# yg838457845/ORB_SLAM2-Chinese-annotation

Measured on AMD Instinct MI355X. Metric: frames/sec (extract+match) at 1241×376, 1000 feat/frame; 1/2/4/8 GPU, higher is better.
Workload: dtype u8; 1 GPU; C4: 1241x376 KITTI-shaped synthetic stream, 1000 feat/frame, SearchByProjection vs 5000-point local map per frame; distinct_frames_per_gpu=8192, frames_per_launch=1024, parallelism=single rank; no collective (one process, one GPU)

## Files before the change

orb_slam2-chinese-annotation_amd/csrc/matcher_kernels.hip:

```cpp
#include <algorithm>
#include <cmath>

#include "matcher_common.h"

__global__ __launch_bounds__(256) void k_hamming_batch(const uint8_t* __restrict__ a,
                                                       const uint8_t* __restrict__ b, int n,
                                                       int32_t* __restrict__ out) {
  const int i = blockIdx.x * blockDim.x + threadIdx.x;
  if (i >= n) return;
  out[i] = hamming256(load_desc(a + (size_t)i * 32), load_desc(b + (size_t)i * 32));
}

#define GB_LDS_KEYS 8192
__global__ __launch_bounds__(64) void k_grid_build(const orb_keypoint_t* __restrict__ keys,
                                                   const int32_t* __restrict__ nkeys, int kpStride,
                                                   float minX, float minY, float invW, float invH,
                                                   int32_t* __restrict__ cellStart,
                                                   int32_t* __restrict__ cellIdx,
                                                   const uint8_t* __restrict__ locked,
                                                   const float* __restrict__ uright,
                                                   uint4* __restrict__ staged) {
  __shared__ __attribute__((aligned(16))) int cnt[GRID_CELLS + 4];
  const int p = blockIdx.x, lane = threadIdx.x;
  const int n = max(nkeys[p], 0);
// ... 361 lines not shown
#pragma unroll
      for (int k = 1; k < 4; ++k)
        if (ix0 + k > nMaxCellX) len[k] = 0;
      const int c1 = len[0], c2 = c1 + len[1], c3 = c2 + len[2], total = c3 + len[3];
      const int o1 = lo[1] - c1, o2 = lo[2] - c2, o3 = lo[3] - c3;
      for (int t = 0; t < total; ++t) {
        const int j = t + (t < c1 ? lo[0] : t < c2 ? o1 : t < c3 ? o2 : o3);
        const uint4 E = gKp[j];
        const int oct = (int)((E.z >> 24) & 0x7Fu);
        if (oct < minL || oct > maxL) continue;
        const float dx = __uint_as_float(E.x) - x, dy = __uint_as_float(E.y) - y;
        if (!(fabsf(dx) < rs && fabsf(dy) < rs) || (E.z >> 31) != 0) continue;
        const float ur = __uint_as_float(E.w);
        if (ur > 0 && fabsf(mp.proj_xr - ur) > rs) continue;
        fn((E.z & 0xFFFFFFu) | ((uint32_t)oct << 24));
      }
    }
  };
  if (staged) {
    int nq = 0;
    uint32_t qe[PROJ_QB];
#pragma unroll
    for (int k = 0; k < PROJ_QB; ++k) qe[k] = 0;
    auto flush = [&](int cnt) {
      ulonglong4 dd[PROJ_QB];
#pragma unroll
      for (int k = 0; k < PROJ_QB; ++k)
        dd[k] = load_desc(D + (size_t)((k < cnt ? qe[k] : qe[0]) & 0xFFFFFFu) * 32);
#pragma unroll
      for (int k = 0; k < PROJ_QB; ++k) {
        if (k >= cnt) break;
        const int dist = hamming256(q, dd[k]);
        if (dist >= 256) continue;
        ++count;
        top.insert(pack_cand((int)(qe[k] & 0xFFFFFFu), dist, (int)(qe[k] >> 24)), dist);
      }
    };
    walk([&](uint32_t qv) {
#pragma unroll
      for (int k = 0; k < PROJ_QB; ++k) qe[k] = nq == k ? qv : qe[k];
      if (++nq == PROJ_QB) {
        flush(PROJ_QB);
        nq = 0;
      }
    });
    if (nq) flush(nq);
  } else {
    for_features_in_area(K, cs, ci, P, mp.proj_x, mp.proj_y, rs, lvl - 1, lvl,
                         [&](int idx, const orb_keypoint_t& kp) {
                           visit(idx, kp.octave, LK && LK[idx], UR ? UR[idx] : -1.0f);
                         });
  }
  top.store(topk + mg * TOPK);
  int slot = -1;
  if (count > TOPK && count <= OVF_CAP && P.ovf) {
    slot = ovf_alloc(P.ovfCtr + p, P.gen);
    if (slot >= OVF_SLOTS) slot = -1;
  }
  if (slot >= 0) {
    uint32_t* lst = P.ovf + ((size_t)p * OVF_SLOTS + slot) * OVF_CAP;
    int n = 0;
    auto put = [&](int idx, int oct) {
      const int dist = hamming256(q, load_desc(D + (size_t)idx * 32));
      if (dist < 256 && n < OVF_CAP) lst[n++] = pack_cand(idx, dist, oct);
    };
    if (staged)
      walk([&](uint32_t qv) { put((int)(qv & 0xFFFFFFu), (int)(qv >> 24)); });
    else
      for_features_in_area(K, cs, ci, P, mp.proj_x, mp.proj_y, rs, lvl - 1, lvl,
                           [&](int idx, const orb_keypoint_t& kp) {
                             if ((LK && LK[idx]) || (UR && UR[idx] > 0 && fabsf(mp.proj_xr - UR[idx]) > rs))
                               return;
                             put(idx, kp.octave);
                           });
  }
  ncand[mg] = count | (mp.has_obs ? NC_OBS : 0) | ((slot + 1) << NC_SLOT_SHIFT);
  }
}

__device__ __forceinline__ bool lock_test(const uint32_t* bm, int idx) {
  return (bm[idx >> 5] >> (idx & 31)) & 1u;
}


template <int NW>
__global__ __launch_bounds__(64 * NW) void k_proj_resolve(
    const orb_keypoint_t* __restrict__ keys, const uint8_t* __restrict__ desc,
    const float* __restrict__ uright, const uint8_t* __restrict__ locked,
    const int32_t* __restrict__ nkeys, int kpStride, const orb_mp_track_t* __restrict__ mps,
    const uint8_t* __restrict__ mpDesc, const int32_t* __restrict__ nmps, int mpStride,
    const int32_t* __restrict__ cellStart, const int32_t* __restrict__ cellIdx, ProjParams P,
    const uint32_t* __restrict__ topk, const int32_t* __restrict__ ncand,
    int32_t* __restrict__ kpMatch, int32_t* __restrict__ nmatches) {
  constexpr int W = 64 * NW, CHUNK = 256 * NW;
  extern __shared__ __attribute__((aligned(16))) uint32_t dyn[];
  __shared__ uint4 cTop[CHUNK];
  __shared__ int cN[CHUNK];
  __shared__ uint8_t cObs[CHUNK];
  __shared__ int sFirst[NW], sCount[NW];
  __shared__ int sSlow;
  const int p = blockIdx.x, t = threadIdx.x, lane = t & 63, wv = t >> 6;
  const int n = nkeys[p], M = nmps[p];
  const int words = (kpStride + 31) >> 5;
  uint32_t* bm = dyn;
  int* claimBy = (int*)(dyn + ((words + 3) & ~3));
  for (int i = t; i < words; i += W) bm[i] = 0u;
  for (int i = t; i < kpStride; i += W) claimBy[i] = W;
  int32_t* km = kpMatch + (size_t)p * kpStride;
  for (int i = t; i < n; i += W) km[i] = -1;
  __syncthreads();
  const float nnratio = P.nnratio;
  const size_t pbase = (size_t)p * mpStride;
  int matches = 0;
  int start = 0;
  int cb = -CHUNK;
  while (start < M) {
    if (start + W > cb + CHUNK && cb + CHUNK < M) {
      cb = start;
      __syncthreads();
      for (int j = t; j < CHUNK; j += W) {
        const int m = cb + j;
        if (m < M) {
          cTop[j] = *reinterpret_cast<const uint4*>(topk + (pbase + m) * TOPK);
          const int v = ncand[pbase + m];
          cN[j] = v;
          cObs[j] = nc_obs(v);
        }
      }
      __syncthreads();
    }
    const int m = start + t;
    const bool active = m < M;
    int nc = -1, ncRaw = -1;
    uint32_t e[TOPK];
    bool hasObs = false;
    if (active) {
      const int j = m - cb;
      ncRaw = cN[j];
      nc = nc_count(ncRaw);
      const uint4 t4 = cTop[j];
      e[0] = t4.x; e[1] = t4.y; e[2] = t4.z; e[3] = t4.w;
      hasObs = cObs[j] != 0;
    }
    int bestDist = 256, bestLevel = -1, bestDist2 = 256, bestLevel2 = -1, bestIdx = -1;
    int consumed = 0, found = 0;
    if (nc > 0) {
      const int avail = nc < TOPK ? nc : TOPK;
      for (int j = 0; j < avail && found < 2; ++j) {
        ++consumed;
        const int idx = cand_idx(e[j]);
        if (lock_test(bm, idx)) continue;
        if (found == 0) {
          bestDist = cand_dist(e[j]);
          bestLevel = cand_oct(e[j]);
          bestIdx = idx;
        } else {
          bestDist2 = cand_dist(e[j]);
          bestLevel2 = cand_oct(e[j]);
        }
        ++found;
      }
    }
    const bool slow = nc > TOPK && found < 2;
    const int slowSlot = nc_slot(ncRaw);
    bool accept = false;
    if (nc > 0 && !slow && bestDist <= 100)
      accept = !(bestLevel == bestLevel2 && (float)bestDist > nnratio * (float)bestDist2);
    const bool locks = accept && hasObs;
    if (locks) atomicMin(&claimBy[bestIdx], t);
    __syncthreads();
    bool conflict = false;
    for (int q = 0; q < consumed; ++q) conflict |= claimBy[cand_idx(e[q])] < t;
    const unsigned long long bad = __ballot(active && (conflict || (slow && t > 0)));
    if (lane == 0) sFirst[wv] = bad ? wv * 64 + (int)__builtin_ctzll(bad) : W;
    if (t == 0) sSlow = active && slow;
    __syncthreads();
    if (locks) claimBy[bestIdx] = W;
    int commit = W;
#pragma unroll
    for (int i = 0; i < NW; ++i) commit = min(commit, sFirst[i]);
    if (sSlow) {
      if (t == 0 && slowSlot >= 0) {
        const uint32_t* lst = ovf_list(P, p, slowSlot);
        int bd = 256, bl = -1, bd2 = 256, bl2 = -1, bi = -1;
        for (int j = 0; j < nc; ++j) {
          const uint32_t ce = lst[j];
          const int idx = cand_idx(ce);
          if (lock_test(bm, idx)) continue;
          const int dist = cand_dist(ce);
          if (dist < bd) {
            bd2 = bd; bd = dist; bl2 = bl; bl = cand_oct(ce); bi = idx;
          } else if (dist < bd2) {
            bl2 = cand_oct(ce); bd2 = dist;
          }
        }
        if (bd <= 100 && !(bl == bl2 && (float)bd > nnratio * (float)bd2)) {
          atomicMax(&km[bi], m);
          if (cObs[m - cb]) bm[bi >> 5] |= 1u << (bi & 31);
          ++matches;
        }
      } else if (t == 0) {
        const size_t mg = pbase + m;
        const orb_mp_track_t mp = mps[mg];
        const int lvl = mp.level;
        float r = (double)mp.view_cos > 0.998 ? 2.5f : 4.0f;
        if (P.th != 1.0f) r *= P.th;
        const float rs = r * P.scale[lvl];
        const orb_keypoint_t* K = keys + (size_t)p * kpStride;
        const uint8_t* D = desc + (size_t)p * kpStride * 32;
        const uint8_t* LK = locked ? locked + (size_t)p * kpStride : nullptr;
        const float* UR = uright ? uright + (size_t)p * kpStride : nullptr;
        const ulonglong4 qd = load_desc(mpDesc + mg * 32);
        int bd = 256, bl = -1, bd2 = 256, bl2 = -1, bi = -1;
        for_features_in_area(K, cellStart + (size_t)p * (GRID_CELLS + 1),
                             cellIdx + (size_t)p * kpStride, P, mp.proj_x, mp.proj_y, rs,
                             lvl - 1, lvl, [&](int idx, const orb_keypoint_t& kp) {
                               if ((LK && LK[idx]) || lock_test(bm, idx)) return;
                               if (UR && UR[idx] > 0) {
                                 const float er = fabsf(mp.proj_xr - UR[idx]);
                                 if (er > r * P.scale[lvl]) return;
                               }
                               const int dist = hamming256(qd, load_desc(D + (size_t)idx * 32));
                               if (dist < bd) {
                                 bd2 = bd; bd = dist; bl2 = bl; bl = kp.octave; bi = idx;
                               } else if (dist < bd2) {
                                 bl2 = kp.octave; bd2 = dist;
                               }
                             });
        if (bd <= 100 && !(bl == bl2 && (float)bd > nnratio * (float)bd2)) {
          atomicMax(&km[bi], m);
          if (mp.has_obs) bm[bi >> 5] |= 1u << (bi & 31);
          ++matches;
        }
      }
      commit = 1;
    } else {
      if (t < commit && accept) {
        atomicMax(&km[bestIdx], m);
        if (locks) atomicOr(&bm[bestIdx >> 5], 1u << (bestIdx & 31));
      }
      matches += __popcll(__ballot(t < commit && accept));
    }
    __syncthreads();
    start += commit;
  }
  if (lane == 0) sCount[wv] = matches;
  __syncthreads();
  if (t == 0) {
    int tot = 0;
#pragma unroll
    for (int i = 0; i < NW; ++i) tot += sCount[i];
    nmatches[p] = tot;
  }
}


__device__ __forceinline__ void lds_barrier() {
  __builtin_amdgcn_fence(__ATOMIC_RELEASE, "workgroup", "local");
  __builtin_amdgcn_s_barrier();
  __builtin_amdgcn_fence(__ATOMIC_ACQUIRE, "workgroup", "local");
}

__device__ __noinline__ int fp_slow(int m, const int* cur, const orb_mp_track_t* mpp,
                                    const uint8_t* mpd, const orb_keypoint_t* K, const uint8_t* D,
                                    const uint8_t* LK, const float* UR, const int32_t* cs,
                                    const int32_t* ci, const ProjParams P, const uint32_t* lst,
                                    int nl) {
  if (lst) {
    uint32_t e[OVF_CAP];
#pragma unroll
    for (int j = 0; j < OVF_CAP; j += 4) {
      const uint4 v = *reinterpret_cast<const uint4*>(lst + j);
      e[j] = v.x; e[j + 1] = v.y; e[j + 2] = v.z; e[j + 3] = v.w;
    }
    int cv[OVF_CAP];
#pragma unroll
    for (int j = 0; j < OVF_CAP; ++j) cv[j] = cur[cand_idx(j < nl ? e[j] : e[0])];
    int bestDist = 256, bestLevel = -1, bestDist2 = 256, bestLevel2 = -1, bestIdx = -1;
#pragma unroll
    for (int j = 0; j < OVF_CAP; ++j) {
      if (j >= nl || cv[j] < m) continue;
      const int dist = cand_dist(e[j]);
      if (dist < bestDist) {
        bestDist2 = bestDist; bestDist = dist;
        bestLevel2 = bestLevel; bestLevel = cand_oct(e[j]); bestIdx = cand_idx(e[j]);
      } else if (dist < bestDist2) {
        bestLevel2 = cand_oct(e[j]); bestDist2 = dist;
      }
    }
    const bool accept = bestIdx >= 0 && bestDist <= 100 &&
                        !(bestLevel == bestLevel2 && (float)bestDist > P.nnratio * (float)bestDist2);
    return accept ? bestIdx : -1;
  }
  const orb_mp_track_t mp = *mpp;
  const int lvl = mp.level;
  float r = (double)mp.view_cos > 0.998 ? 2.5f : 4.0f;
  if (P.th != 1.0f) r *= P.th;
  const float rs = r * P.scale[lvl];
  const ulonglong4 qd = load_desc(mpd);
  int bestDist = 256, bestLevel = -1, bestDist2 = 256, bestLevel2 = -1, bestIdx = -1;
  for_features_in_area(K, cs, ci, P, mp.proj_x, mp.proj_y, rs, lvl - 1, lvl,
                       [&](int idx, const orb_keypoint_t& kp) {
                         if ((LK && LK[idx]) || cur[idx] < m) return;
                         if (UR && UR[idx] > 0) {
                           const float er = fabsf(mp.proj_xr - UR[idx]);
                           if (er > rs) return;
                         }
                         const int dist = hamming256(qd, load_desc(D + (size_t)idx * 32));
                         if (dist < bestDist) {
                           bestDist2 = bestDist; bestDist = dist;
                           bestLevel2 = bestLevel; bestLevel = kp.octave; bestIdx = idx;
                         } else if (dist < bestDist2) {
                           bestLevel2 = kp.octave; bestDist2 = dist;
                         }
                       });
  const bool accept = bestIdx >= 0 && bestDist <= 100 &&
                      !(bestLevel == bestLevel2 && (float)bestDist > P.nnratio * (float)bestDist2);
  return accept ? bestIdx : -1;
}

__device__ __forceinline__ int fp_choose(const uint32_t (&e)[TOPK], int nc, int m, const int* cur,
                                         const orb_mp_track_t* mpp, const uint8_t* mpd,
                                         const orb_keypoint_t* K, const uint8_t* D,
                                         const uint8_t* LK, const float* UR, const int32_t* cs,
                                         const int32_t* ci, const ProjParams& P,
                                         const uint32_t* lst) {
  int bestDist = 256, bestLevel = -1, bestDist2 = 256, bestLevel2 = -1, bestIdx = -1;
  int found = 0;
  const int avail = nc < TOPK ? nc : TOPK;
  int cv[TOPK];
#pragma unroll
  for (int j = 0; j < TOPK; ++j) cv[j] = cur[cand_idx(j < avail ? e[j] : e[0])];
  bool taken[TOPK];
#pragma unroll
  for (int j = 0; j < TOPK; ++j) taken[j] = j < avail ? cv[j] < m : true;
#pragma unroll
  for (int j = 0; j < TOPK; ++j) {
    const bool use = found < 2 && !taken[j];
    if (use && found == 0) {
      bestDist = cand_dist(e[j]); bestLevel = cand_oct(e[j]); bestIdx = cand_idx(e[j]);
    } else if (use) {
      bestDist2 = cand_dist(e[j]); bestLevel2 = cand_oct(e[j]);
    }
    found += use ? 1 : 0;
// ... 364 lines not shown
    hipLaunchKernelGGL((k_proj_candidates<PROJ_WG, false, PROJ_PPT_SMALL>), grid, dim3(wg), lds, s, keys,
                       desc, uright, locked, kpStride, nkeys, mps, mpDesc, nmps, mpStride, cellStart,
                       cellIdx, sg, stageCap, P, topk, ncand);
  return hipGetLastError();
}

#ifndef RESOLVE_FP_T
#define RESOLVE_FP_T 1024
#endif
#ifndef RESOLVE_FP_W
#define RESOLVE_FP_W 1024
#endif
#define RESOLVE_FP_MIN_MAP 20000
#define RESOLVE_FP_FEW 8
#ifndef RESOLVE_AUTO_FP
#define RESOLVE_AUTO_FP 0
#endif
#ifndef RESOLVE_W1_MIN
#define RESOLVE_W1_MIN 128
#endif
#define RESOLVE_FP_LDS_MAX (160 * 1024 - 1024)

int orb_k_proj_resolve_kernel(int nproblems, int kpStride, int mpStride, int schedule) {
  const bool fpFits = (size_t)kpStride * 12 <= RESOLVE_FP_LDS_MAX;
  if (fpFits) {
    if (schedule == ORB_RESOLVE_JACOBI) return ORB_RESOLVE_KERNEL_JACOBI;
    if (schedule == ORB_RESOLVE_FIXED_POINT) return ORB_RESOLVE_KERNEL_FIXED_POINT;
    if (schedule == ORB_RESOLVE_AUTO && (mpStride >= RESOLVE_FP_MIN_MAP || nproblems <= RESOLVE_FP_FEW ||
                                         RESOLVE_AUTO_FP))
      return ORB_RESOLVE_KERNEL_FIXED_POINT;
  }
  if (mpStride >= RESOLVE_FP_MIN_MAP) return ORB_RESOLVE_KERNEL_PREFIX_W8;
  return nproblems >= RESOLVE_W1_MIN ? ORB_RESOLVE_KERNEL_PREFIX_W1 : ORB_RESOLVE_KERNEL_PREFIX_W4;
}

size_t orb_k_proj_jacobi_bytes(int kpStride, int mpStride, int nproblems, int schedule) {
  if (orb_k_proj_resolve_kernel(nproblems, kpStride, mpStride, schedule) != ORB_RESOLVE_KERNEL_JACOBI)
    return 0;
  return (size_t)jacobi_stride(kpStride, mpStride) * 4 * (size_t)nproblems;
}

hipError_t orb_k_proj_resolve(const orb_keypoint_t* keys, const uint8_t* desc,
                              const float* uright, const uint8_t* locked, const int32_t* nkeys,
                              int kpStride, const orb_mp_track_t* mps, const uint8_t* mpDesc,
                              const int32_t* nmps, int mpStride, const int32_t* cellStart,
                              const int32_t* cellIdx, const void* params, const uint32_t* topk,
                              const int32_t* ncand, int32_t* kpMatch, int32_t* nmatches,
                              int nproblems, int schedule, int jacobiRounds, int32_t* jacScratch,
                              hipStream_t s) {
  const ProjParams P = *(const ProjParams*)params;
  if (nproblems <= 0) return hipSuccess;
  const int kern = orb_k_proj_resolve_kernel(nproblems, kpStride, mpStride, schedule);
  if (kern == ORB_RESOLVE_KERNEL_FIXED_POINT || kern == ORB_RESOLVE_KERNEL_JACOBI) {
    const size_t ldsFp = (size_t)kpStride * 12;
    if (ldsFp > 64 * 1024) {
      hipError_t e = hipFuncSetAttribute((const void*)k_proj_resolve_fp<RESOLVE_FP_T, RESOLVE_FP_W / RESOLVE_FP_T>,
                                         hipFuncAttributeMaxDynamicSharedMemorySize, (int)ldsFp);
      if (e != hipSuccess) return e;
    }
    const int32_t* done = nullptr;
    long long doneStride = 0;
    if (kern == ORB_RESOLVE_KERNEL_JACOBI) {
      if (!jacScratch) return hipErrorInvalidValue;
      const int R = std::max(1, std::min(48, jacobiRounds));
      const long long js = jacobi_stride(kpStride, mpStride);
      const int initN = std::max(3 * kpStride, R + 1);
      hipLaunchKernelGGL(k_proj_jacobi_init, dim3((initN + JAC_T - 1) / JAC_T, nproblems), dim3(JAC_T),
                         0, s, jacScratch, js, kpStride, R, nkeys, kpMatch, nmatches);
      const dim3 g((std::max(mpStride, 1) + JAC_T * JAC_PPT - 1) / (JAC_T * JAC_PPT), nproblems);
      for (int r = 0; r <= R; ++r)
        hipLaunchKernelGGL(k_proj_jacobi<JAC_PPT>, g, dim3(JAC_T), 0, s, keys, desc, uright, locked,
                           kpStride, mps, mpDesc, nmps, mpStride, cellStart, cellIdx, P, topk, ncand,
                           kpMatch, nmatches, jacScratch, js, r, R);
      done = jacScratch + R;
      doneStride = js;
    }
    hipLaunchKernelGGL((k_proj_resolve_fp<RESOLVE_FP_T, RESOLVE_FP_W / RESOLVE_FP_T>), dim3(nproblems), dim3(RESOLVE_FP_T),
                       ldsFp, s, keys, desc,
                       uright, locked, nkeys, kpStride, mps, mpDesc, nmps, mpStride, cellStart,
                       cellIdx, P, topk, ncand, kpMatch, nmatches, done, doneStride);
    return hipGetLastError();
  }
  const size_t words = (size_t)((kpStride + 31) / 32);
  const size_t lds = ((words + 3) & ~(size_t)3) * 4 + (size_t)kpStride * 4;
  if (kern == ORB_RESOLVE_KERNEL_PREFIX_W8)
    hipLaunchKernelGGL(k_proj_resolve<8>, dim3(nproblems), dim3(512), lds, s, keys, desc, uright,
                       locked, nkeys, kpStride, mps, mpDesc, nmps, mpStride, cellStart, cellIdx,
                       P, topk, ncand, kpMatch, nmatches);
  else if (kern == ORB_RESOLVE_KERNEL_PREFIX_W1)
    hipLaunchKernelGGL(k_proj_resolve<1>, dim3(nproblems), dim3(64), lds, s, keys, desc, uright,
                       locked, nkeys, kpStride, mps, mpDesc, nmps, mpStride, cellStart, cellIdx,
                       P, topk, ncand, kpMatch, nmatches);
  else
    hipLaunchKernelGGL(k_proj_resolve<4>, dim3(nproblems), dim3(256), lds, s, keys, desc, uright,
                       locked, nkeys, kpStride, mps, mpDesc, nmps, mpStride, cellStart, cellIdx,
                       P, topk, ncand, kpMatch, nmatches);
  return hipGetLastError();
}

size_t orb_k_proj_params_size(void) { return sizeof(ProjParams); }

size_t orb_k_proj_ovf_bytes(int nproblems) {
  return (size_t)std::max(nproblems, 1) * OVF_SLOTS * OVF_CAP * 4;
}


}

struct StereoParams {
  int nLevels;
  float bf, fx;
  int w[ORB_MAX_LEVELS], h[ORB_MAX_LEVELS];
  int strideL[ORB_MAX_LEVELS], strideR[ORB_MAX_LEVELS];
  float scale[ORB_MAX_LEVELS], invScale[ORB_MAX_LEVELS];
};

struct StereoPairLevels {
  const uint8_t* L[ORB_MAX_LEVELS];
  const uint8_t* R[ORB_MAX_LEVELS];
};

__global__ __launch_bounds__(1024) void k_stereo_rows(const orb_keypoint_t* __restrict__ rkeys,
                                                      const int32_t* __restrict__ nright,
                                                      int kpStride, StereoParams P,
                                                      int32_t* __restrict__ rowStart,
                                                      int32_t* __restrict__ rowIdx, int rowCap) {
  extern __shared__ int cnt[];
  __shared__ int tmp[17];
  const int pair = blockIdx.x, t = threadIdx.x, T = blockDim.x;
  const int H = P.h[0], NR = nright[pair];
  const orb_keypoint_t* K = rkeys + (size_t)pair * kpStride;
  for (int i = t; i <= H; i += T) cnt[i] = 0;
  __syncthreads();
  auto band = [&](const orb_keypoint_t& kp, int* lo, int* hi) {
    const float r = 2.0f * P.scale[kp.octave];
    *lo = max((int)floorf(kp.y - r), 0);
    *hi = min((int)ceilf(kp.y + r), H - 1);
  };
  for (int iR = t; iR < NR; iR += T) {
    int lo, hi;
    band(K[iR], &lo, &hi);
    for (int yi = lo; yi <= hi; ++yi) atomicAdd(&cnt[yi], 1);
  }
  __syncthreads();
  {
    const int n = H + 1, per = (n + T - 1) / T, b = min(t * per, n), e = min(b + per, n);
    int sum = 0;
    for (int i = b; i < e; ++i) sum += cnt[i];
    int total;
    int ex = block_excl_scan(sum, tmp, &total);
    for (int i = b; i < e; ++i) {
      const int v = cnt[i];
      cnt[i] = ex;
      ex += v;
    }
    __syncthreads();
  }
  int32_t* rs = rowStart + (size_t)pair * (H + 1);
  for (int i = t; i <= H; i += T) rs[i] = cnt[i];
  __syncthreads();
  int32_t* ri = rowIdx + (size_t)pair * 2 * rowCap;
  float* rx = reinterpret_cast<float*>(ri + rowCap);
  for (int iR = t; iR < NR; iR += T) {
    const orb_keypoint_t kp = K[iR];
    int lo, hi;
    band(kp, &lo, &hi);
    const int e = iR | (kp.octave << 24);
    for (int yi = lo; yi <= hi; ++yi) {
      const int pos = atomicAdd(&cnt[yi], 1);
      if (pos < rowCap) {
        ri[pos] = e;
        rx[pos] = kp.x;
      }
    }
  }
}

__global__ __launch_bounds__(256) void k_stereo_match(
    const orb_keypoint_t* __restrict__ lkeys, const uint8_t* __restrict__ ldesc,
// ... 819 lines not shown
```

orb_slam2-chinese-annotation_amd/csrc/runtime.cpp:

```cpp
#include <hip/hip_runtime.h>
#include <math.h>
#include <stdint.h>
#include <stdio.h>
#include <stdlib.h>
#include <string.h>

#include <algorithm>
#include <chrono>
#include <mutex>
#include <shared_mutex>
#include <cmath>
#include <vector>

#include "../../include/orb_abi.h"
#include "orb_plan.h"
#include "orb_synth.h"

extern "C" {
hipError_t orb_k_upload_constants(hipStream_t s);
hipError_t orb_k_upload_umax(const int* umax16, hipStream_t s);
hipError_t orb_k_pyr_resize(const uint8_t* src, long long srcImgPitch, int srcStride, int sw,
                            int sh, uint8_t* dst, long long dstImgPitch, int dstStride, int dw,
                            int dh, const int* xofs, const void* alpha, const int* yofs,
                            const void* beta, int mode, int nimg, hipStream_t s);
// ... 1423 lines not shown
      orb_k_frustum_params_size() != sizeof(FrustumParamsHost) ||
      orb_k_init_params_size() != sizeof(InitParamsHost) ||
      orb_k_pp_params_size() != sizeof(PPParamsHost) ||
      orb_k_tri_params_size() != sizeof(TriParamsHost))
    return ORB_EINVAL;
  orb_matcher* m = new orb_matcher();
  m->device = device;
  m->prof.nStages = 3;
  m->prof.names[0] = "k_grid_build";
  m->prof.names[1] = "k_proj_candidates";
  m->prof.names[2] = "k_proj_resolve";
  for (int i = 0; i < 3; ++i) m->prof.launchesPerCall[i] = 1;
  hipSetDevice(device);
  if (create_own_stream(&m->stream) != hipSuccess) {
    delete m;
    return ORB_EDEVICE;
  }
  if (hipEventCreateWithFlags(&m->evLast, hipEventDisableTiming) != hipSuccess) {
    hipStreamDestroy(m->stream);
    delete m;
    return ORB_EDEVICE;
  }
  *out = m;
  return ORB_OK;
}

void orb_matcher_destroy(orb_matcher_t* m) {
  if (!m) return;
  hipSetDevice(m->device);
  hipStreamSynchronize(m->stream);
  if (m->lastStream) hipEventSynchronize(m->evLast);
  DevBuf* bufs[] = {&m->dKeys, &m->dDesc, &m->dUr, &m->dLocked, &m->dNKeys, &m->dMps,
                    &m->dMpDesc, &m->dNMps, &m->dCellStart, &m->dCellIdx, &m->dTopk,
                    &m->dNcand, &m->dKpMatch, &m->dNMatch, &m->dA, &m->dB, &m->dOut, &m->dJac,
                    &m->dRKeys, &m->dRDesc, &m->dNR, &m->dPyr, &m->dPairLv, &m->dDepth,
                    &m->dSad, &m->dStRowStart, &m->dStRowIdx, &m->dProjStage, &m->dBowA, &m->dBowB, &m->dBowC, &m->dBowD, &m->dBowE,
                    &m->dBowF, &m->dBowG, &m->dBowH, &m->dBowI, &m->dBowJ, &m->dBowK,
                    &m->dMapPts, &m->dPose, &m->dTracks, &m->dNInView, &m->dK1, &m->dD1,
                    &m->dK2, &m->dD2, &m->dN1, &m->dN2, &m->dPrev, &m->dList, &m->dM12,
                    &m->dOffs, &m->dObsDesc, &m->dBest, &m->dBestDesc, &m->dInitQ,
                    &m->dInitStage, &m->dInitCounts, &m->dOvf, &m->dOvfCtr};
  for (DevBuf* b : bufs) b->release();
  m->hPyr.release();
  m->hIn.release();
  m->hOutM.release();
  m->dIn.release();
  for (DevBuf& b : m->sx) b.release();
  m->prof.destroy();
  hipStreamDestroy(m->stream);
  hipEventDestroy(m->evLast);
  delete m;
}

void* orb_matcher_stream(orb_matcher_t* m) { return m ? (void*)m->stream : nullptr; }

orb_status_t orb_hamming_batch(orb_matcher_t* m, const uint8_t* d_a, const uint8_t* d_b, int n,
                               int32_t* d_dist, void* stream) {
  if (!m || n < 0 || (n > 0 && (!d_a || !d_b || !d_dist))) return ORB_EINVAL;
  hipSetDevice(m->device);
  HIP_TRY(orb_k_hamming(d_a, d_b, n, d_dist, stream ? (hipStream_t)stream : m->stream));
  return ORB_OK;
}

static ProjParamsHost proj_params(float min_x, float max_x, float min_y, float max_y,
                                  int n_levels, const float* scale, float th, float nnratio) {
  ProjParamsHost P;
  memset(&P, 0, sizeof(P));
  P.minX = min_x;
  P.minY = min_y;
  P.invW = (float)ORB_GRID_COLS / (max_x - min_x);
  P.invH = (float)ORB_GRID_ROWS / (max_y - min_y);
  P.th = th;
  P.nnratio = nnratio;
  P.nLevels = n_levels;
  for (int i = 0; i < n_levels && i < ORB_MAX_LEVELS; ++i) P.scale[i] = scale[i];
  return P;
}

static orb_status_t ovf_pool(orb_matcher_t* m, int nproblems, ProjParamsHost& P, hipStream_t s) {
  orb_status_t st;
  if ((st = m->dOvf.ensure(orb_k_proj_ovf_bytes(nproblems)))) return st;
  const size_t oldBytes = m->dOvfCtr.bytes;
  if ((st = m->dOvfCtr.ensure((size_t)std::max(nproblems, 1) * 4))) return st;
  if (m->dOvfCtr.bytes != oldBytes) HIP_TRY(hipMemsetAsync(m->dOvfCtr.p, 0, m->dOvfCtr.bytes, s));
  m->ovfGen = m->ovfGen % 4095u + 1u;
  P.ovf = m->dOvf.as<uint32_t>();
  P.ovfCtr = m->dOvfCtr.as<uint32_t>();
  P.gen = m->ovfGen;
  return ORB_OK;
}

orb_status_t orb_match_projection_local_batch(
    orb_matcher_t* m, int n_problems, const orb_keypoint_t* d_keys, const uint8_t* d_desc,
    const int32_t* d_nkeys, const uint8_t* d_locked, int kp_stride,
    const orb_mp_track_t* d_mps, const uint8_t* d_mp_desc, const int32_t* d_nmps,
    int mp_stride, float min_x, float max_x, float min_y, float max_y, int n_levels,
    const float* scale_factors, float th, float nnratio, int32_t* d_kp_match,
    int32_t* d_nmatches, void* stream) {
  if (!m || n_problems < 0 || kp_stride <= 0 || mp_stride < 0 || !scale_factors ||
      n_levels <= 0 || n_levels > ORB_MAX_LEVELS || kp_stride >= (1 << 19) || !(max_x > min_x) ||
      !(max_y > min_y))
    return ORB_EINVAL;
  if (n_problems == 0) return ORB_OK;
  std::lock_guard<std::mutex> g(m->mu);
  hipSetDevice(m->device);
  hipStream_t s = stream ? (hipStream_t)stream : m->stream;
  CallOrder order(m->evLast, &m->lastStream, s);
  if (order.status) return order.status;
  ProjParamsHost P =
      proj_params(min_x, max_x, min_y, max_y, n_levels, scale_factors, th, nnratio);
  orb_status_t st;
  if ((st = ovf_pool(m, n_problems, P, s))) return st;
  if ((st = m->dCellStart.ensure((size_t)n_problems * (ORB_GRID_COLS * ORB_GRID_ROWS + 1) * 4)))
    return st;
  if ((st = m->dCellIdx.ensure((size_t)n_problems * kp_stride * 4))) return st;
  if ((st = m->dTopk.ensure((size_t)n_problems * std::max(mp_stride, 1) * 16))) return st;
  if ((st = m->dNcand.ensure((size_t)n_problems * std::max(mp_stride, 1) * 4))) return st;
  const bool stage = kp_stride <= orb_k_grid_stage_max();
  if (stage && (st = m->dProjStage.ensure((size_t)n_problems * kp_stride * 16))) return st;
  const size_t jb = orb_k_proj_jacobi_bytes(kp_stride, mp_stride, n_problems, m->resolveSchedule);
  if (jb && (st = m->dJac.ensure(jb))) return st;
  StageProfiler& pf = m->prof;
  std::vector<hipEvent_t>* ev = pf.begin_call();
  PROF_REC(ev, pf.t0(ev), s);
  PROF_REC(ev, pf.b(ev, 0), s);
  if (stage)
    HIP_TRY(orb_k_grid_build_staged(d_keys, d_nkeys, d_locked, nullptr, kp_stride, P.minX, P.minY,
                                    P.invW, P.invH, m->dCellStart.as<int32_t>(),
                                    m->dCellIdx.as<int32_t>(), m->dProjStage.p, n_problems, s));
  else
    HIP_TRY(orb_k_grid_build(d_keys, d_nkeys, kp_stride, P.minX, P.minY, P.invW, P.invH,
                             m->dCellStart.as<int32_t>(), m->dCellIdx.as<int32_t>(), n_problems,
                             s));
  PROF_REC(ev, pf.e(ev, 0), s);
  PROF_REC(ev, pf.b(ev, 1), s);
  HIP_TRY(orb_k_proj_candidates(d_keys, d_desc, nullptr, d_locked, kp_stride, d_nkeys, d_mps, d_mp_desc,
                                d_nmps, mp_stride, mp_stride, m->dCellStart.as<int32_t>(),
                                m->dCellIdx.as<int32_t>(), stage ? m->dProjStage.p : nullptr,
                                &P, m->dTopk.as<uint32_t>(),
                                m->dNcand.as<int32_t>(), n_problems, s));
  PROF_REC(ev, pf.e(ev, 1), s);
  PROF_REC(ev, pf.b(ev, 2), s);
  HIP_TRY(orb_k_proj_resolve(d_keys, d_desc, nullptr, d_locked, d_nkeys, kp_stride, d_mps,
                             d_mp_desc, d_nmps, mp_stride, m->dCellStart.as<int32_t>(),
                             m->dCellIdx.as<int32_t>(), &P, m->dTopk.as<uint32_t>(),
                             m->dNcand.as<int32_t>(), d_kp_match, d_nmatches, n_problems,
                             m->resolveSchedule, m->jacobiRounds, m->dJac.as<int32_t>(), s));
  PROF_REC(ev, pf.e(ev, 2), s);
  PROF_REC(ev, pf.t1(ev), s);
  return ORB_OK;
}

orb_status_t orb_matcher_set_resolve(orb_matcher_t* m, int schedule, int jacobi_rounds) {
  if (!m || schedule < ORB_RESOLVE_AUTO || schedule > ORB_RESOLVE_JACOBI ||
      (schedule == ORB_RESOLVE_JACOBI && (jacobi_rounds < 1 || jacobi_rounds > 48)))
    return ORB_EINVAL;
  std::lock_guard<std::mutex> g(m->mu);
  m->resolveSchedule = schedule;
  if (schedule == ORB_RESOLVE_JACOBI) m->jacobiRounds = jacobi_rounds;
  return ORB_OK;
}

orb_status_t orb_matcher_resolve_kernel(orb_matcher_t* m, int n_problems, int kp_stride,
                                        int mp_stride, int* kernel) {
  if (!m || !kernel || n_problems <= 0 || kp_stride <= 0 || mp_stride < 0) return ORB_EINVAL;
  std::lock_guard<std::mutex> g(m->mu);
  *kernel = orb_k_proj_resolve_kernel(n_problems, kp_stride, std::max(mp_stride, 1),
// ... 1592 lines not shown
```

Before: 346,000 frames/s.

## Pipeline resolve kernel with register prefetch ring, LDS kpMatch and wave-level sync

Restructures the prefix-resolve kernel so that candidate top-k and counts are staged through an LDS ring buffer filled from register prefetches several blocks ahead, replacing the stop-and-refill chunk loads. When LDS allows, the per-keypoint match array is kept in LDS and written out at the end. For single-wave configurations the workgroup barriers are replaced by wave barriers and ballots. The lock and claim lookups are unrolled into independent loads. It also resets the overflow counters when the generation wraps. The cost is higher register and LDS pressure, which may reduce occupancy.

```diff
diff --git a/orb_slam2-chinese-annotation_amd/csrc/matcher_kernels.hip b/orb_slam2-chinese-annotation_amd/csrc/matcher_kernels.hip
--- a/orb_slam2-chinese-annotation_amd/csrc/matcher_kernels.hip
+++ b/orb_slam2-chinese-annotation_amd/csrc/matcher_kernels.hip
@@ -467,8 +467,66 @@
   return (bm[idx >> 5] >> (idx & 31)) & 1u;
 }
 
+__device__ __forceinline__ void lds_barrier() {
+  __builtin_amdgcn_fence(__ATOMIC_RELEASE, "workgroup", "local");
+  __builtin_amdgcn_s_barrier();
+  __builtin_amdgcn_fence(__ATOMIC_ACQUIRE, "workgroup", "local");
+}
 
 template <int NW>
+__device__ __forceinline__ void round_sync() {
+  if constexpr (NW == 1) {
+    __builtin_amdgcn_fence(__ATOMIC_ACQ_REL, "wavefront");
+    __builtin_amdgcn_wave_barrier();
+  } else {
+    lds_barrier();
+  }
+}
+
+__device__ __forceinline__ int prefix_slow(const uint32_t* bm, const orb_mp_track_t* mpp,
+                                        const uint8_t* mpd, const orb_keypoint_t* K,
+                                        const uint8_t* D, const uint8_t* LK, const float* UR,
+                                        const int32_t* cs, const int32_t* ci, const ProjParams& P,
+                                        const uint32_t* lst, int nl) {
+  int bd = 256, bl = -1, bd2 = 256, bl2 = -1, bi = -1;
+  if (lst) {
+    for (int j = 0; j < nl; ++j) {
+      const uint32_t ce = lst[j];
+      const int idx = cand_idx(ce);
+      if (lock_test(bm, idx)) continue;
+      const int dist = cand_dist(ce);
+      if (dist < bd) {
+        bd2 = bd; bd = dist; bl2 = bl; bl = cand_oct(ce); bi = idx;
+      } else if (dist < bd2) {
+        bl2 = cand_oct(ce); bd2 = dist;
+      }
+    }
+  } else {
+    const orb_mp_track_t mp = *mpp;
+    const int lvl = mp.level;
+    float r = (double)mp.view_cos > 0.998 ? 2.5f : 4.0f;
+    if (P.th != 1.0f) r *= P.th;
+    const float rs = r * P.scale[lvl];
+    const ulonglong4 qd = load_desc(mpd);
+    for_features_in_area(K, cs, ci, P, mp.proj_x, mp.proj_y, rs, lvl - 1, lvl,
+                         [&](int idx, const orb_keypoint_t& kp) {
+                           if ((LK && LK[idx]) || lock_test(bm, idx)) return;
+                           if (UR && UR[idx] > 0) {
+                             const float er = fabsf(mp.proj_xr - UR[idx]);
+                             if (er > rs) return;
+                           }
+                           const int dist = hamming256(qd, load_desc(D + (size_t)idx * 32));
+                           if (dist < bd) {
+                             bd2 = bd; bd = dist; bl2 = bl; bl = kp.octave; bi = idx;
+                           } else if (dist < bd2) {
+                             bl2 = kp.octave; bd2 = dist;
+                           }
+                         });
+  }
+  return bd <= 100 && !(bl == bl2 && (float)bd > P.nnratio * (float)bd2) ? bi : -1;
+}
+
+template <int NW, bool KM_LDS>
 __global__ __launch_bounds__(64 * NW) void k_proj_resolve(
     const orb_keypoint_t* __restrict__ keys, const uint8_t* __restrict__ desc,
     const float* __restrict__ uright, const uint8_t* __restrict__ locked,
@@ -477,11 +535,10 @@
     const int32_t* __restrict__ cellStart, const int32_t* __restrict__ cellIdx, ProjParams P,
     const uint32_t* __restrict__ topk, const int32_t* __restrict__ ncand,
     int32_t* __restrict__ kpMatch, int32_t* __restrict__ nmatches) {
-  constexpr int W = 64 * NW, CHUNK = 256 * NW;
+  constexpr int W = 64 * NW, RING = 4, CHUNK = RING * W, AHEAD = 4;
   extern __shared__ __attribute__((aligned(16))) uint32_t dyn[];
   __shared__ uint4 cTop[CHUNK];
   __shared__ int cN[CHUNK];
-  __shared__ uint8_t cObs[CHUNK];
   __shared__ int sFirst[NW], sCount[NW];
   __shared__ int sSlow;
   const int p = blockIdx.x, t = threadIdx.x, lane = t & 63, wv = t >> 6;
@@ -489,132 +546,123 @@
   const int words = (kpStride + 31) >> 5;
   uint32_t* bm = dyn;
   int* claimBy = (int*)(dyn + ((words + 3) & ~3));
+  int32_t* km = KM_LDS ? (int32_t*)(claimBy + kpStride) : kpMatch + (size_t)p * kpStride;
   for (int i = t; i < words; i += W) bm[i] = 0u;
   for (int i = t; i < kpStride; i += W) claimBy[i] = W;
-  int32_t* km = kpMatch + (size_t)p * kpStride;
   for (int i = t; i < n; i += W) km[i] = -1;
-  __syncthreads();
   const float nnratio = P.nnratio;
   const size_t pbase = (size_t)p * mpStride;
+  auto load = [&](uint4& e, int& nc, int b) {
+    const size_t mg = pbase + (size_t)min(b * W + t, M - 1);
+    const uint32_t* tp = topk + mg * TOPK;
+    e = make_uint4(tp[0], tp[1], tp[2], tp[3]);
+    nc = ncand[mg];
+  };
+  auto store = [&](const uint4& e, int nc, int b) {
+    const int j = (b * W + t) & (CHUNK - 1);
+    cTop[j] = e;
+    cN[j] = nc;
+  };
+  uint4 pfTop[AHEAD];
+  int pfN[AHEAD];
+#pragma unroll
+  for (int c = 0; c < AHEAD; ++c) {
+    pfTop[c] = make_uint4(0u, 0u, 0u, 0u);
+    pfN[c] = -1;
+  }
+  int pfb = RING;
+  if (M > 0) {
+    uint4 inTop[RING];
+    int inN[RING];
+#pragma unroll
+    for (int k = 0; k < RING; ++k) load(inTop[k], inN[k], k);
+#pragma unroll
+    for (int k = 0; k < RING; ++k) store(inTop[k], inN[k], k);
+#pragma unroll
+    for (int c = 0; c < AHEAD; ++c)
+      load(pfTop[(RING + c) % AHEAD], pfN[(RING + c) % AHEAD], RING + c);
+  }
+  if constexpr (KM_LDS)
+    round_sync<NW>();
+  else
+    __syncthreads();
   int matches = 0;
   int start = 0;
-  int cb = -CHUNK;
-  while (start < M) {
-    if (start + W > cb + CHUNK && cb + CHUNK < M) {
-      cb = start;
-      __syncthreads();
-      for (int j = t; j < CHUNK; j += W) {
-        const int m = cb + j;
-        if (m < M) {
-          cTop[j] = *reinterpret_cast<const uint4*>(topk + (pbase + m) * TOPK);
-          const int v = ncand[pbase + m];
-          cN[j] = v;
-          cObs[j] = nc_obs(v);
-        }
-      }
-      __syncthreads();
-    }
+  auto round = [&]() {
     const int m = start + t;
     const bool active = m < M;
     int nc = -1, ncRaw = -1;
-    uint32_t e[TOPK];
-    bool hasObs = false;
+    uint32_t e[TOPK] = {0u, 0u, 0u, 0u};
     if (active) {
-      const int j = m - cb;
+      const int j = m & (CHUNK - 1);
       ncRaw = cN[j];
       nc = nc_count(ncRaw);
       const uint4 t4 = cTop[j];
       e[0] = t4.x; e[1] = t4.y; e[2] = t4.z; e[3] = t4.w;
-      hasObs = cObs[j] != 0;
-    }
+    }
+    const bool hasObs = nc_obs(ncRaw);
     int bestDist = 256, bestLevel = -1, bestDist2 = 256, bestLevel2 = -1, bestIdx = -1;
     int consumed = 0, found = 0;
-    if (nc > 0) {
-      const int avail = nc < TOPK ? nc : TOPK;
-      for (int j = 0; j < avail && found < 2; ++j) {
-        ++consumed;
-        const int idx = cand_idx(e[j]);
-        if (lock_test(bm, idx)) continue;
-        if (found == 0) {
-          bestDist = cand_dist(e[j]);
-          bestLevel = cand_oct(e[j]);
-          bestIdx = idx;
-        } else {
-          bestDist2 = cand_dist(e[j]);
-          bestLevel2 = cand_oct(e[j]);
-        }
-        ++found;
-      }
+    const int avail = nc < TOPK ? (nc > 0 ? nc : 0) : TOPK;
+    uint32_t lw[TOPK];
+#pragma unroll
+    for (int j = 0; j < TOPK; ++j) lw[j] = bm[(j < avail ? cand_idx(e[j]) : 0) >> 5];
+#pragma unroll
+    for (int j = 0; j < TOPK; ++j) {
+      const bool look = j < avail && found < 2;
+      const int idx = cand_idx(e[j]);
+      const bool use = look && !((lw[j] >> (idx & 31)) & 1u);
+      if (use && found == 0) {
+        bestDist = cand_dist(e[j]); bestLevel = cand_oct(e[j]); bestIdx = idx;
+      } else if (use) {
+        bestDist2 = cand_dist(e[j]); bestLevel2 = cand_oct(e[j]);
+      }
+      consumed += look ? 1 : 0;
+      found += use ? 1 : 0;
     }
     const bool slow = nc > TOPK && found < 2;
-    const int slowSlot = nc_slot(ncRaw);
     bool accept = false;
     if (nc > 0 && !slow && bestDist <= 100)
       accept = !(bestLevel == bestLevel2 && (float)bestDist > nnratio * (float)bestDist2);
     const bool locks = accept && hasObs;
     if (locks) atomicMin(&claimBy[bestIdx], t);
-    __syncthreads();
+    round_sync<NW>();
+    int cl[TOPK];
+#pragma unroll
+    for (int q = 0; q < TOPK; ++q) cl[q] = claimBy[q < consumed ? cand_idx(e[q]) : 0];
     bool conflict = false;
-    for (int q = 0; q < consumed; ++q) conflict |= claimBy[cand_idx(e[q])] < t;
+#pragma unroll
+    for (int q = 0; q < TOPK; ++q) conflict |= q < consumed && cl[q] < t;
     const unsigned long long bad = __ballot(active && (conflict || (slow && t > 0)));
-    if (lane == 0) sFirst[wv] = bad ? wv * 64 + (int)__builtin_ctzll(bad) : W;
-    if (t == 0) sSlow = active && slow;
-    __syncthreads();
+    int commit;
+    bool anySlow;
+    if constexpr (NW == 1) {
+      commit = bad ? (int)__builtin_ctzll(bad) : W;
+      anySlow = (__ballot(active && slow) & 1ull) != 0;
+      round_sync<NW>();
+    } else {
+      if (lane == 0) sFirst[wv] = bad ? wv * 64 + (int)__builtin_ctzll(bad) : W;
+      if (t == 0) sSlow = active && slow;
+      round_sync<NW>();
+      commit = W;
+#pragma unroll
+      for (int i = 0; i < NW; ++i) commit = min(commit, sFirst[i]);
+      anySlow = sSlow != 0;
+    }
     if (locks) claimBy[bestIdx] = W;
-    int commit = W;
-#pragma unroll
-    for (int i = 0; i < NW; ++i) commit = min(commit, sFirst[i]);
-    if (sSlow) {
-      if (t == 0 && slowSlot >= 0) {
-        const uint32_t* lst = ovf_list(P, p, slowSlot);
-        int bd = 256, bl = -1, bd2 = 256, bl2 = -1, bi = -1;
-        for (int j = 0; j < nc; ++j) {
-          const uint32_t ce = lst[j];
-          const int idx = cand_idx(ce);
-          if (lock_test(bm, idx)) continue;
-          const int dist = cand_dist(ce);
-          if (dist < bd) {
-            bd2 = bd; bd = dist; bl2 = bl; bl = cand_oct(ce); bi = idx;
-          } else if (dist < bd2) {
-            bl2 = cand_oct(ce); bd2 = dist;
-          }
-        }
-        if (bd <= 100 && !(bl == bl2 && (float)bd > nnratio * (float)bd2)) {
+    if (anySlow) {
+      if (t == 0) {
+        const int slot = nc_slot(ncRaw);
+        const int bi = prefix_slow(bm, mps + pbase + m, mpDesc + (pbase + m) * 32,
+                                   keys + (size_t)p * kpStride, desc + (size_t)p * kpStride * 32,
+                                   locked ? locked + (size_t)p * kpStride : nullptr,
+                                   uright ? uright + (size_t)p * kpStride : nullptr,
+                                   cellStart + (size_t)p * (GRID_CELLS + 1),
+                                   cellIdx + (size_t)p * kpStride, P,
+                                   slot >= 0 ? ovf_list(P, p, slot) : nullptr, nc);
+        if (bi >= 0) {
           atomicMax(&km[bi], m);
-          if (cObs[m - cb]) bm[bi >> 5] |= 1u << (bi & 31);
-          ++matches;
-        }
-      } else if (t == 0) {
-        const size_t mg = pbase + m;
-        const orb_mp_track_t mp = mps[mg];
-        const int lvl = mp.level;
-        float r = (double)mp.view_cos > 0.998 ? 2.5f : 4.0f;
-        if (P.th != 1.0f) r *= P.th;
-        const float rs = r * P.scale[lvl];
-        const orb_keypoint_t* K = keys + (size_t)p * kpStride;
-        const uint8_t* D = desc + (size_t)p * kpStride * 32;
-        const uint8_t* LK = locked ? locked + (size_t)p * kpStride : nullptr;
-        const float* UR = uright ? uright + (size_t)p * kpStride : nullptr;
-        const ulonglong4 qd = load_desc(mpDesc + mg * 32);
-        int bd = 256, bl = -1, bd2 = 256, bl2 = -1, bi = -1;
-        for_features_in_area(K, cellStart + (size_t)p * (GRID_CELLS + 1),
-                             cellIdx + (size_t)p * kpStride, P, mp.proj_x, mp.proj_y, rs,
-                             lvl - 1, lvl, [&](int idx, const orb_keypoint_t& kp) {
-                               if ((LK && LK[idx]) || lock_test(bm, idx)) return;
-                               if (UR && UR[idx] > 0) {
-                                 const float er = fabsf(mp.proj_xr - UR[idx]);
-                                 if (er > r * P.scale[lvl]) return;
-                               }
-                               const int dist = hamming256(qd, load_desc(D + (size_t)idx * 32));
-                               if (dist < bd) {
-                                 bd2 = bd; bd = dist; bl2 = bl; bl = kp.octave; bi = idx;
-                               } else if (dist < bd2) {
-                                 bl2 = kp.octave; bd2 = dist;
-                               }
-                             });
-        if (bd <= 100 && !(bl == bl2 && (float)bd > nnratio * (float)bd2)) {
-          atomicMax(&km[bi], m);
-          if (mp.has_obs) bm[bi >> 5] |= 1u << (bi & 31);
+          if (hasObs) bm[bi >> 5] |= 1u << (bi & 31);
           ++matches;
         }
       }
@@ -626,8 +674,24 @@
       }
       matches += __popcll(__ballot(t < commit && accept));
     }
-    __syncthreads();
+    round_sync<NW>();
     start += commit;
+  };
+  static_assert(RING % AHEAD == 0, "block RING is held in pfTop[0]");
+  while (start < M) {
+#pragma unroll
+    for (int c = 0; c < AHEAD; ++c) {
+      while (start < min(M, (pfb - RING + 1) * W)) round();
+      if (start >= M) goto done;
+      store(pfTop[c], pfN[c], pfb);
+      load(pfTop[c], pfN[c], pfb + AHEAD);
+      ++pfb;
+    }
+  }
+done:
+  if constexpr (KM_LDS) {
+    int32_t* out = kpMatch + (size_t)p * kpStride;
+    for (int i = t; i < n; i += W) out[i] = km[i];
   }
   if (lane == 0) sCount[wv] = matches;
   __syncthreads();
@@ -639,12 +703,6 @@
   }
 }
 
-
-__device__ __forceinline__ void lds_barrier() {
-  __builtin_amdgcn_fence(__ATOMIC_RELEASE, "workgroup", "local");
-  __builtin_amdgcn_s_barrier();
-  __builtin_amdgcn_fence(__ATOMIC_ACQUIRE, "workgroup", "local");
-}
 
 __device__ __noinline__ int fp_slow(int m, const int* cur, const orb_mp_track_t* mpp,
                                     const uint8_t* mpd, const orb_keypoint_t* K, const uint8_t* D,
@@ -1175,19 +1233,22 @@
     return hipGetLastError();
   }
   const size_t words = (size_t)((kpStride + 31) / 32);
-  const size_t lds = ((words + 3) & ~(size_t)3) * 4 + (size_t)kpStride * 4;
-  if (kern == ORB_RESOLVE_KERNEL_PREFIX_W8)
-    hipLaunchKernelGGL(k_proj_resolve<8>, dim3(nproblems), dim3(512), lds, s, keys, desc, uright,
-                       locked, nkeys, kpStride, mps, mpDesc, nmps, mpStride, cellStart, cellIdx,
-                       P, topk, ncand, kpMatch, nmatches);
-  else if (kern == ORB_RESOLVE_KERNEL_PREFIX_W1)
-    hipLaunchKernelGGL(k_proj_resolve<1>, dim3(nproblems), dim3(64), lds, s, keys, desc, uright,
-                       locked, nkeys, kpStride, mps, mpDesc, nmps, mpStride, cellStart, cellIdx,
-                       P, topk, ncand, kpMatch, nmatches);
-  else
-    hipLaunchKernelGGL(k_proj_resolve<4>, dim3(nproblems), dim3(256), lds, s, keys, desc, uright,
-                       locked, nkeys, kpStride, mps, mpDesc, nmps, mpStride, cellStart, cellIdx,
-                       P, topk, ncand, kpMatch, nmatches);
+  const int nw = kern == ORB_RESOLVE_KERNEL_PREFIX_W8 ? 8 : kern == ORB_RESOLVE_KERNEL_PREFIX_W1 ? 1 : 4;
+  size_t lds = ((words + 3) & ~(size_t)3) * 4 + (size_t)kpStride * 4;
+  const bool kmLds = lds + (size_t)kpStride * 4 + (size_t)nw * 5200 <= 64 * 1024;
+  if (kmLds) lds += (size_t)kpStride * 4;
+#define RESOLVE_LAUNCH(NW, KM)                                                                     \
+  hipLaunchKernelGGL((k_proj_resolve<NW, KM>), dim3(nproblems), dim3(64 * NW), lds, s, keys, desc, \
+                     uright, locked, nkeys, kpStride, mps, mpDesc, nmps, mpStride, cellStart,      \
+                     cellIdx, P, topk, ncand, kpMatch, nmatches)
+  if (nw == 8) {
+    if (kmLds) RESOLVE_LAUNCH(8, true); else RESOLVE_LAUNCH(8, false);
+  } else if (nw == 1) {
+    if (kmLds) RESOLVE_LAUNCH(1, true); else RESOLVE_LAUNCH(1, false);
+  } else {
+    if (kmLds) RESOLVE_LAUNCH(4, true); else RESOLVE_LAUNCH(4, false);
+  }
+#undef RESOLVE_LAUNCH
   return hipGetLastError();
 }
 
diff --git a/orb_slam2-chinese-annotation_amd/csrc/runtime.cpp b/orb_slam2-chinese-annotation_amd/csrc/runtime.cpp
--- a/orb_slam2-chinese-annotation_amd/csrc/runtime.cpp
+++ b/orb_slam2-chinese-annotation_amd/csrc/runtime.cpp
@@ -1529,7 +1529,8 @@
   if ((st = m->dOvf.ensure(orb_k_proj_ovf_bytes(nproblems)))) return st;
   const size_t oldBytes = m->dOvfCtr.bytes;
   if ((st = m->dOvfCtr.ensure((size_t)std::max(nproblems, 1) * 4))) return st;
-  if (m->dOvfCtr.bytes != oldBytes) HIP_TRY(hipMemsetAsync(m->dOvfCtr.p, 0, m->dOvfCtr.bytes, s));
+  if (m->dOvfCtr.bytes != oldBytes || m->ovfGen >= 4095u)
+    HIP_TRY(hipMemsetAsync(m->dOvfCtr.p, 0, m->dOvfCtr.bytes, s));
   m->ovfGen = m->ovfGen % 4095u + 1u;
   P.ovf = m->dOvf.as<uint32_t>();
   P.ovfCtr = m->dOvfCtr.as<uint32_t>();
```

Measured after the change: 356,500 frames/s (median of 6 runs). 3.0% higher.
